# atenpas/agile_grasp

Measured on AMD Instinct MI355X. Metric: grasp hypotheses/sec on 300k-pt cloud @2000 samples, higher is better.
Workload: dtype f64

## Files before the change

### agile_grasp_amd/csrc/agh_internal.h

```cpp
#pragma once

#include <hip/hip_runtime.h>
#include <stdint.h>

#include <string>
#include <vector>

#include "agh.h"

namespace agh
{

constexpr int kBboxBlocks = 128;
constexpr int kCountBlocks = 2048;
constexpr int kGridMargin = 2;
constexpr int kCellCap = 1 << 21;
constexpr int kCellStride = kCellCap + 4;
constexpr int kMaxRows = 128;
constexpr int kNumSums = 37;
constexpr int kSumStride = 40;
constexpr int kSlots = 8;
constexpr int kImageWords = 250;
constexpr int kBigListGrid = 512;
constexpr int kSweepWg4MinSamples = 4096;
constexpr int64_t kNormalsChunk = 16384;

struct GridDesc
{
  double mn[3];
  double cell;
  double inv_cell;
  int dim[3];
  int ncell;
  unsigned open;
  unsigned ticket;
};

constexpr int kMaxClouds = 64;
struct GridView
{
  const GridDesc* desc;
  const int* cell_start;
  const float4* sorted;
  const int* cloud_off;
  int n_clouds;
};

struct HandGeom
{
  double finger_width, hand_outer_diameter, hand_depth, hand_height, init_bite;
  double cam_origin[2][3];
  double cos_a[8], sin_a[8];
  double fs[20];
  double thr[40];
  int n_thr;
  int lo_idx[20], hi_idx[20];
  double depths[16];
  double backs[16];
  double boxy[16];
  int n_depths;
  double cos_antipodal;
  double xlut_lo, xlut_scale;
  double ylut_lo, ylut_scale;
  unsigned char xlut[1024];
  unsigned char ylut[64];
  int x_probes, y_probes;
};
constexpr int kLutProbe = 4;

struct HogTablesDev
{
  float mag0[9], mag1[9];
  int bin0[9], bin1[9];
  alignas(16) float coef[9][12];
  int pix_x[256], pix_y[256];
  float pix_wcell[256][4];
};

enum SampleStatus : int
{
  kStatusOk = 0,
  kStatusOverflow = 1,
  kStatusDegenerate = 2,
  kStatusRows = 3,
  kStatusBadIndex = 4,
  kStatusSkipped = 5
};
constexpr int32_t kSampleSkip = INT32_MIN;
constexpr int kBigCap = 4096;
constexpr int kHugeCap = 6144;
constexpr int64_t kHugeEntries = 1ll << 21;

constexpr unsigned long long kVoxMaxWords = 1ull << 28;
struct VoxDesc
{
  unsigned mn_enc[2][3], mx_enc[2][3];
  double mn[2][3];
  int dim[2][3];
  unsigned long long bits[2], word_ofs[2], n_words;
  long long n_kept[2], n_vox[2];
  int error;
};
struct VoxWorkspace
{
  double lo[3], hi[3];
};

struct Comm;

struct HostMirror
{
  agh_hypothesis* rec;
  int64_t cap;
  int64_t* hdr;
};

struct LocalizeState
{
  bool active = false;
  bool repeated = false;
  bool deferred = false;
  bool classify = false, with_sequential = false, explicit_samples = false;
  int64_t S = 0, nv = 0;
  int32_t min_inliers = 0;
  double min_length = 0.0, x1 = 0.0, x2 = 0.0;
  agh_localize_params lp{};
  const float* d_raw = nullptr;
  int64_t dev_stride = 0, n_raw = 0;
  bool staged = false;
  const float* staged_src = nullptr;
  int64_t staged_stride = 0, staged_n = 0;
};

struct PlaneState;

struct Ctx
{
  agh_params p;
  HandGeom geom;
  int device = 0;
  hipStream_t stream = nullptr;
  hipEvent_t copy_done = nullptr;
  hipEvent_t copy_gate = nullptr;
  hipEvent_t xyz_copied = nullptr;
  bool cam_copy_on_copy_stream = false;
  hipStream_t copy_stream = nullptr;
  bool copy_stream_failed = false;
  std::string err;

  int64_t n = 0;
  const float* d_xyz = nullptr;
  int64_t stride_floats = 3;
  const int32_t* d_cam = nullptr;
  float* own_xyz = nullptr;
  int32_t* own_cam = nullptr;
  int64_t own_cap = 0;
  int64_t own_cap_floats = 0;
  int32_t* d_idx_own = nullptr;
  int64_t idx_cap = 0;
  uint8_t* h_pin = nullptr;
  int64_t h_pin_samples = 0, h_pin_records = 0;
  HostMirror mirror{ nullptr, 0, nullptr };
  uint8_t* h_pin_handles = nullptr;
  int64_t h_pin_handles_cap = 0;
  bool handles_sequential = false;
  uint8_t* h_pin_keep = nullptr;
  int64_t h_pin_keep_cap = 0;

  VoxDesc* d_vox_desc = nullptr;
  uint8_t* d_vox_code = nullptr;
  int* d_vox_blk = nullptr;
  int* d_vox_blk2 = nullptr;
  long long* d_vox_total = nullptr;
  unsigned* d_vox_bitmap = nullptr;
  int64_t vox_bitmap_cap = 0;
// ... 650 lines not shown
```

### agile_grasp_amd/csrc/api.hip

```cpp
#include "agh_internal.h"

#include <algorithm>
#include <atomic>
#include <cmath>
#include <cstdio>
#include <cstdlib>
#include <cstring>

using namespace agh;


namespace
{
thread_local std::string g_create_error;
std::atomic<int32_t> g_epoch{ 0 };
}

namespace agh
{
int32_t next_epoch()
{
  int32_t e;
  do
    e = (int32_t) ((uint32_t) g_epoch.fetch_add(1) + 1u) & 0x7fffffff;
// ... 960 lines not shown
  }
  int* h_counts = reinterpret_cast<int*>(c->h_pin_handles);
  agh_hypothesis* h_hands = reinterpret_cast<agh_hypothesis*>(c->h_pin_handles + 256);
  agh_handle* h_handles = reinterpret_cast<agh_handle*>(h_hands + c->h_pin_handles_cap);
  int32_t* h_idx = reinterpret_cast<int32_t*>(h_handles + c->h_pin_handles_cap);
  if (n_hands > 0)
  {
    std::memcpy(h_hands, hands, sizeof(agh_hypothesis) * (size_t) n_hands);
    HIPCHK(c, hipMemcpyAsync(c->d_h_hands, h_hands, sizeof(agh_hypothesis) * n_hands, hipMemcpyHostToDevice, c->stream));
  }
  const HandleMirror hm{ h_handles, (int) c->h_pin_handles_cap, h_idx, (int) c->h_pin_handles_cap, h_counts };
  for (int attempt = 0; attempt < 2; attempt++)
  {
    h_counts[0] = h_counts[1] = h_counts[2] = h_counts[3] = 0;
    timing_begin(c, c->stream);
    const bool with_sequential = c->handles_sequential;
    const int rc = handle_search(c, n_hands, x1, x2, min_inliers, min_length, c->stream, hm, with_sequential);
    timing_mark(c, "handle_search", c->stream);
    if (rc != AGH_OK)
    {
      c->err = "handle search launch failed";
      return rc;
    }
    HIPCHK(c, hipStreamSynchronize(c->stream));
    const bool declined = h_counts[3] != 0;
    c->handles_sequential = declined;
    if (!declined || with_sequential)
      break;
  }
  const int* counts = h_counts;
  if (counts[2])
  {
    c->err = "agh_find_handles: a seed hand has more than 2048 inliers";
    return AGH_ERR_CAPACITY;
  }
  *n_handles_out = counts[0];
  if (counts[0] > handle_cap || counts[1] > idx_cap)
  {
    c->err = "agh_find_handles: output buffers too small";
    return AGH_ERR_CAPACITY;
  }
  if (counts[0] > 0)
  {
    std::memcpy(handles_out, h_handles, sizeof(agh_handle) * (size_t) counts[0]);
    std::memcpy(inlier_idx_out, h_idx, sizeof(int32_t) * (size_t) counts[1]);
  }
  return AGH_OK;
}

int agh_get_cloud(agh_ctx* ctx, float* xyz_out, int32_t* cam_out, int64_t cap)
{
  if (!ctx || cap < 0)
    return AGH_ERR_INVALID_ARGUMENT;
  Ctx* c = &ctx->c;
  if (refuse_mid_chain(c, "agh_get_cloud"))
    return AGH_ERR_STATE;
  if (!c->has_cloud)
  {
    c->err = "agh_get_cloud: no cloud set";
    return AGH_ERR_NO_CLOUD;
  }
  HIPCHK(c, hipSetDevice(c->device));
  HIPCHK(c, hipDeviceSynchronize());
  const int64_t k = std::min<int64_t>(cap, c->n);
  if (k > 0 && xyz_out)
    HIPCHK(c, hipMemcpy2D(xyz_out, 12, c->d_xyz, (size_t) c->stride_floats * 4, 12, (size_t) k, hipMemcpyDeviceToHost));
  if (k > 0 && cam_out)
  {
    if (c->d_cam)
      HIPCHK(c, hipMemcpy(cam_out, c->d_cam, sizeof(int32_t) * k, hipMemcpyDeviceToHost));
    else
      std::memset(cam_out, 0, sizeof(int32_t) * k);
  }
  return (int) std::min<int64_t>(c->n, 0x7fffffff);
}

int agh_find_hands_device(agh_ctx* ctx, const int32_t* d_sample_idx, int64_t n_samples, int calculates_antipodal,
  agh_hypothesis* d_out, int64_t cap, int64_t* d_n_out, void* hip_stream)
{
  if (!ctx)
    return AGH_ERR_INVALID_ARGUMENT;
  Ctx* c = &ctx->c;
  if (refuse_mid_chain(c, "agh_find_hands"))
    return AGH_ERR_STATE;
  if (!c->has_cloud)
  {
    c->err = "agh_find_hands: no cloud set";
    return AGH_ERR_NO_CLOUD;
  }
  if (n_samples < 0 || n_samples > (1 << 24) || (n_samples > 0 && (!d_sample_idx || !d_out)) || !d_n_out || cap < 0)
  {
    c->err = "agh_find_hands: bad arguments";
    return AGH_ERR_INVALID_ARGUMENT;
  }
  HIPCHK(c, hipSetDevice(c->device));
  hipStream_t st = hip_stream ? (hipStream_t) hip_stream : c->stream;
  HIPCHK(c, order_after_cloud(c, st));
  const int64_t S = n_samples;
  const int64_t chunk = kNormalsChunk;
  int rc = ensure_call_buffers(c, std::max<int64_t>(S, calculates_antipodal ? std::min<int64_t>(c->n, chunk) : 0));
  if (rc != AGH_OK)
    return rc;
  const bool rand_mode = c->p.normals_mode == AGH_NORMALS_RAND50;
  if (rand_mode)
  {
    rc = ensure_draws(c, 50 * (S + (calculates_antipodal ? c->n : 0)), st);
    if (rc != AGH_OK)
      return rc;
  }
  timing_begin(c, st);
  c->zero_flags_pending = true;
  c->last_s = S;
  c->epoch = next_epoch();
  c->last_nout = -1;
  c->last_cap = cap;
  c->d_out_last = d_out;
  c->d_nout_last = d_n_out;
  if (S == 0 || c->n == 0)
  {
    HIPCHK(c, hipMemsetAsync(c->d_flags, 0, 8 * sizeof(int32_t), st));
    c->zero_flags_pending = false;
    HIPCHK(c, hipMemsetAsync(d_n_out, 0, sizeof(int64_t), st));
    c->last_s = 0;
    return AGH_OK;
  }
  if (calculates_antipodal)
  {
    if (c->n > c->normals_cap)
    {
      if ((rc = dev_alloc(c, &c->d_normals, (size_t) c->n * 3)))
        return rc;
      c->normals_cap = c->n;
    }
    HIPCHK(c, hipMemsetAsync(c->d_normals, 0, sizeof(double) * 3 * c->n, st));
    if ((rc = normals_pass(c, 0, c->n, st)) != AGH_OK)
    {
      c->err = "normals pass launch failed";
      return rc;
    }
    c->has_normals = true;
  }
  rc = taubin_frames(c, d_sample_idx, S, c->p.nn_radius_taubin, c->d_frames, c->d_nt, calculates_antipodal != 0, st);
  if (rc != AGH_OK)
  {
    c->err = "taubin launch failed";
    return rc;
  }
  if (c->debug_stop_moments || (c->debug_stop_frame && c->debug_stop_frame < 5))
  {
    HIPCHK(c, hipMemsetAsync(d_n_out, 0, sizeof(int64_t), st));
    return AGH_OK;
  }
#ifdef AGH_DEBUG_HOOKS
  if (std::getenv("AGH_DEBUG_CLOCKS") && !c->d_dbg && hipMalloc((void**) &c->d_dbg, sizeof(long long) * 8 * c->s_cap) != hipSuccess)
    c->d_dbg = nullptr;
#endif
  rc = hand_sweep(c, d_sample_idx, S, calculates_antipodal != 0, st);
  if (rc != AGH_OK)
  {
    c->err = "hand sweep launch failed";
    return rc;
  }
  if (c->debug_stop_sweep && c->debug_stop_sweep < 10)
  {
    HIPCHK(c, hipMemsetAsync(d_n_out, 0, sizeof(int64_t), st));
    return AGH_OK;
  }
  rc = compact_hypotheses(c, S, d_out, cap, d_n_out, st);
  if (rc != AGH_OK)
  {
    c->err = "compaction launch failed";
    return rc;
  }
  return AGH_OK;
}


static int check_flags(Ctx* c, hipStream_t st)
{
  int32_t flags[8];
  HIPCHK(c, hipMemcpyAsync(flags, c->d_flags, sizeof(flags), hipMemcpyDeviceToHost, st));
  HIPCHK(c, hipStreamSynchronize(st));
  return flags_to_status(c, flags);
}

extern "C++" int flags_to_status(Ctx* c, const int32_t* flags_in)
{
  int32_t flags[1] = { flags_in[0] };
  if (flags[0] & kFlagSharded)
  {
    flags[0] &= ~1;
    if (flags[0] & kFlagShardPeerNoCloud)
    {
      c->err = "a rank of the communicator holds no cloud (agh_set_cloud* on every rank first); no list";
      return AGH_ERR_NO_CLOUD;
    }
    if (flags[0] & kFlagShardPeerFailed)
    {
      c->err = "a rank of the communicator could not do its share of the call (its own agh_last_error says why); no list";
      return AGH_ERR_STATE;
    }
    if (flags[0] & kFlagShardHard)
    {
      c->err = "the Taubin neighbourhoods (r = nn_radius_taubin) of more than 4096 points of one launch hold more than 2^21 points in "
               "all; voxelise the cloud (localization.cpp:43) or reduce the radii";
      return AGH_ERR_CAPACITY;
    }
    if (flags[0] & (kFlagShardRetry | kFlagShardRetryHuge))
    {
      c->big_classes = true;
      if (flags[0] & kFlagShardRetryHuge)
        c->huge_classes = true;
      c->err = "a Taubin neighbourhood exceeds the capacity classes launched so far; the contexts of the communicator now launch "
               "the larger classes as well: repeat the call";
      return AGH_ERR_RETRY;
    }
  }
  if ((flags[0] & 1) && !c->big_classes)
  {
    c->big_classes = true;
    c->err = "a Taubin neighbourhood exceeds the first capacity class; the context now launches the larger classes as "
             "well: repeat the call";
    return AGH_ERR_RETRY;
  }
  if ((flags[0] & 1) && !c->huge_classes)
  {
    c->huge_classes = true;
    c->err = "a Taubin neighbourhood exceeds 4096 points; the context now launches the 6144 class as well: repeat the call";
    return AGH_ERR_RETRY;
  }
  if (flags[0] & 1)
  {
    c->err = "the Taubin neighbourhoods (r = nn_radius_taubin) of more than 4096 points of one launch hold more than 2^21 points in "
             "all (the pool of the classes beyond the LDS-resident ones); voxelise the cloud (localization.cpp:43) or reduce the radii";
    return AGH_ERR_CAPACITY;
  }
  if ((flags[0] & 2) && !(flags[0] & 16))
  {
    c->err = "output buffer too small for the hypotheses found";
    return AGH_ERR_CAPACITY;
  }
  if (flags[0] & 4)
  {
    c->err = "a sample index is outside the cloud";
    return AGH_ERR_INVALID_ARGUMENT;
  }
  if (flags[0] & 16)
  {
    c->shard_full_exchange = true;
    c->err = "a rank found more hypotheses than its exchange segment holds; the context now exchanges full-size segments: "
             "repeat the call";
    return AGH_ERR_RETRY;
  }
  return AGH_OK;
}

int agh_find_hands(agh_ctx* ctx, const int32_t* sample_idx, int64_t n_samples, int calculates_antipodal,
  agh_hypothesis* out, int64_t cap, int64_t* n_out)
{
  if (!ctx || !n_out)
    return AGH_ERR_INVALID_ARGUMENT;
  Ctx* c = &ctx->c;
  if (refuse_mid_chain(c, "agh_find_hands"))
    return AGH_ERR_STATE;
  *n_out = 0;
  if (!c->has_cloud)
  {
    c->err = "agh_find_hands: no cloud set";
    return AGH_ERR_NO_CLOUD;
  }
  if (n_samples < 0 || (n_samples > 0 && !sample_idx) || cap < 0 || (cap > 0 && !out))
  {
    c->err = "agh_find_hands: bad arguments";
    return AGH_ERR_INVALID_ARGUMENT;
  }
  for (int64_t i = 0; i < n_samples; i++)
    if (sample_idx[i] < 0 || sample_idx[i] >= c->n)
    {
      c->err = "agh_find_hands: sample index out of range";
      return AGH_ERR_INVALID_ARGUMENT;
    }
  HIPCHK(c, hipSetDevice(c->device));
  int rc = ensure_call_buffers(c, std::max<int64_t>(n_samples, calculates_antipodal ? std::min<int64_t>(c->n, kNormalsChunk) : 0));
  if (rc != AGH_OK)
    return rc;
  if (n_samples > c->idx_cap || !c->d_idx_own)
  {
    if ((rc = dev_alloc(c, &c->d_idx_own, (size_t) std::max<int64_t>(n_samples, 1024))))
      return rc;
    c->idx_cap = std::max<int64_t>(n_samples, 1024);
  }
  int32_t* d_idx = c->d_idx_own;
  if ((rc = ensure_host_staging(c, n_samples, std::min<int64_t>(c->s_cap * 8, kMirrorMaxRecords))) != AGH_OK)
    return rc;
  int64_t* hdr = reinterpret_cast<int64_t*>(c->h_pin);
  int32_t* h_idx = reinterpret_cast<int32_t*>(c->h_pin + kPinHeaderBytes);
  agh_hypothesis* h_rec = reinterpret_cast<agh_hypothesis*>(c->h_pin + kPinHeaderBytes + pin_round(c->h_pin_samples * 4));
  if (n_samples > 0)
  {
    std::memcpy(h_idx, sample_idx, sizeof(int32_t) * (size_t) n_samples);
    HIPCHK(c, hipMemcpyAsync(d_idx, h_idx, sizeof(int32_t) * n_samples, hipMemcpyHostToDevice, c->stream));
  }
  int64_t n = 0;
  for (int attempt = 0; attempt < 3; attempt++)
  {
    if ((rc = ensure_call_buffers(c, std::max<int64_t>(n_samples, calculates_antipodal ? std::min<int64_t>(c->n, kNormalsChunk) : 0))) != AGH_OK)
      return rc;
    hdr[0] = -1;
    hdr[1] = 0;
    c->mirror = HostMirror{ h_rec, c->h_pin_records, hdr };
    rc = agh_find_hands_device(ctx, d_idx, n_samples, calculates_antipodal, c->d_out_own, c->s_cap * 8, c->d_nout,
      c->stream);
    c->mirror = HostMirror{ nullptr, 0, nullptr };
    if (rc == AGH_OK)
    {
      HIPCHK(c, hipStreamSynchronize(c->stream));
      int32_t flags[8] = { 0, 0, 0, 0, 0, 0, 0, 0 };
      if (hdr[0] >= 0)
      {
        n = hdr[0];
        flags[0] = (int32_t) hdr[1] | (n > c->s_cap * 8 ? 2 : 0);
      }
      else
      {
        HIPCHK(c, hipMemcpy(flags, c->d_flags, sizeof(flags), hipMemcpyDeviceToHost));
        HIPCHK(c, hipMemcpy(&n, c->d_nout, sizeof(int64_t), hipMemcpyDeviceToHost));
      }
      rc = flags_to_status(c, flags);
    }
    else
      (void) hipStreamSynchronize(c->stream);
    if (rc != AGH_ERR_RETRY)
      break;
  }
  if (rc != AGH_OK)
    return rc;
  c->last_nout = n;
  *n_out = n;
  if (n > cap)
  {
    c->err = "output buffer too small for the hypotheses found";
    return AGH_ERR_CAPACITY;
  }
  const int64_t from_pin = hdr[0] >= 0 ? std::min<int64_t>(n, c->h_pin_records) : 0;
  if (from_pin > 0)
    std::memcpy(out, h_rec, sizeof(agh_hypothesis) * (size_t) from_pin);
  if (n > from_pin)
    HIPCHK(c, hipMemcpy(out + from_pin, c->d_out_own + from_pin, sizeof(agh_hypothesis) * (size_t) (n - from_pin), hipMemcpyDeviceToHost));
  return AGH_OK;
}

int agh_synchronize(agh_ctx* ctx)
{
  if (!ctx)
    return AGH_ERR_INVALID_ARGUMENT;
  Ctx* c = &ctx->c;
  HIPCHK(c, hipSetDevice(c->device));
  HIPCHK(c, hipDeviceSynchronize());
  if (c->loc.active)
    return AGH_OK;
#ifdef AGH_DEBUG_HOOKS
  if (c->d_dbg && c->last_s > 0 && std::getenv("AGH_DEBUG_CLOCKS"))
  {
    std::vector<long long> h((size_t) c->last_s * 8);
    if (hipMemcpy(h.data(), c->d_dbg, h.size() * 8, hipMemcpyDeviceToHost) == hipSuccess)
      if (FILE* f = std::fopen(std::getenv("AGH_DEBUG_CLOCKS"), "wb"))
      {
        std::fwrite(h.data(), 8, h.size(), f);
        std::fclose(f);
      }
  }
#endif
  const int rc = check_flags(c, c->stream);
  if (rc == AGH_OK && c->last_nout < 0 && c->d_nout_last)
  {
    int64_t n = 0;
    if (hipMemcpy(&n, c->d_nout_last, sizeof(int64_t), hipMemcpyDeviceToHost) == hipSuccess)
      c->last_nout = std::min<int64_t>(n, c->last_cap);
    else
      (void) hipGetLastError();
  }
  return rc;
}

int agh_get_epoch(agh_ctx* ctx, int32_t* epoch, int64_t* n_hyp)
{
  if (!ctx)
    return AGH_ERR_INVALID_ARGUMENT;
  if (refuse_mid_chain(&ctx->c, "agh_get_epoch"))
    return AGH_ERR_STATE;
  if (epoch)
    *epoch = ctx->c.epoch;
  if (n_hyp)
    *n_hyp = ctx->c.last_nout;
  return AGH_OK;
}

int agh_get_frames(agh_ctx* ctx, agh_frame* out, int64_t cap)
{
  if (!ctx || !out)
    return AGH_ERR_INVALID_ARGUMENT;
  Ctx* c = &ctx->c;
  if (refuse_mid_chain(c, "agh_get_frames"))
    return AGH_ERR_STATE;
  const int64_t n = std::min<int64_t>(cap, c->last_s);
  HIPCHK(c, hipDeviceSynchronize());
  if (n > 0)
    HIPCHK(c, hipMemcpy(out, c->d_frames, sizeof(agh_frame) * n, hipMemcpyDeviceToHost));
  return (int) n;
}

int agh_get_neighbor_counts(agh_ctx* ctx, int32_t* n_taubin, int32_t* n_hands, int64_t cap)
{
  if (!ctx)
    return AGH_ERR_INVALID_ARGUMENT;
  Ctx* c = &ctx->c;
  if (refuse_mid_chain(c, "agh_get_neighbor_counts"))
    return AGH_ERR_STATE;
  const int64_t n = std::min<int64_t>(cap, c->last_s);
  HIPCHK(c, hipDeviceSynchronize());
  if (n > 0 && n_taubin)
    HIPCHK(c, hipMemcpy(n_taubin, c->d_nt, sizeof(int32_t) * n, hipMemcpyDeviceToHost));
  if (n > 0 && n_hands)
  {
    if (ball_counts(c, n, c->stream) != AGH_OK)
    {
      c->err = "k_ball_count launch failed";
      return AGH_ERR_HIP;
    }
    HIPCHK(c, hipStreamSynchronize(c->stream));
  }
  if (n > 0 && n_hands)
    HIPCHK(c, hipMemcpy(n_hands, c->d_nh, sizeof(int32_t) * n, hipMemcpyDeviceToHost));
  return (int) n;
}

int agh_get_normals(agh_ctx* ctx, double* normals, int64_t cap_points)
{
  if (!ctx || !normals)
    return AGH_ERR_INVALID_ARGUMENT;
  Ctx* c = &ctx->c;
  if (refuse_mid_chain(c, "agh_get_normals"))
    return AGH_ERR_STATE;
  if (!c->has_normals)
  {
    c->err = "no normals: the last agh_find_hands call did not use calculates_antipodal";
    return AGH_ERR_STATE;
  }
  const int64_t n = std::min<int64_t>(cap_points, c->n);
  HIPCHK(c, hipDeviceSynchronize());
  if (n > 0)
    HIPCHK(c, hipMemcpy(normals, c->d_normals, sizeof(double) * 3 * n, hipMemcpyDeviceToHost));
  return (int) n;
}

int agh_set_profile(agh_ctx* ctx, int32_t level)
{
  if (!ctx || level < 0 || level > 3)
    return AGH_ERR_INVALID_ARGUMENT;
  Ctx* c = &ctx->c;
  if (refuse_mid_chain(c, "agh_set_profile"))
    return AGH_ERR_STATE;
  HIPCHK(c, hipSetDevice(c->device));
  HIPCHK(c, hipDeviceSynchronize());
  c->p.profile = level;
  c->prof_calls = 0;
  c->ev_used = 0;
  c->ev_name.clear();
  return AGH_OK;
}

int agh_get_timing(agh_ctx* ctx, agh_timing* out)
{
  if (!ctx || !out)
    return AGH_ERR_INVALID_ARGUMENT;
  Ctx* c = &ctx->c;
  std::memset(out, 0, sizeof(*out));
  std::memset(c->timing_counts, 0, sizeof(c->timing_counts));
  if (!c->p.profile || c->ev_used < 2)
    return AGH_OK;
  HIPCHK(c, hipEventSynchronize(c->ev[c->ev_used - 1]));
  int k = 0;
  for (int i = 1; i < c->ev_used; i++)
  {
    if (std::strcmp(c->ev_name[i], "start") == 0)
      continue;
    float ms = 0.f;
    if (hipEventElapsedTime(&ms, c->ev[i - 1], c->ev[i]) != hipSuccess)
      ms = 0.f;
    int slot = -1;
    for (int j = 0; j < k; j++)
      if (std::strcmp(out->name[j], c->ev_name[i]) == 0)
        slot = j;
    if (slot < 0)
    {
      if (k >= AGH_TIMING_SLOTS)
        continue;
      slot = k++;
      out->name[slot] = c->ev_name[i];
    }
    out->ms[slot] += ms;
    c->timing_counts[slot]++;
    out->total_ms += ms;
  }
  out->n = k;
  c->ev_used = 0;
  c->ev_name.clear();
  return AGH_OK;
}

int agh_get_timing_counts(agh_ctx* ctx, int32_t* counts, int32_t cap)
{
  if (!ctx || !counts || cap < 0)
    return AGH_ERR_INVALID_ARGUMENT;
  for (int i = 0; i < cap && i < AGH_TIMING_SLOTS; i++)
    counts[i] = ctx->c.timing_counts[i];
  return AGH_OK;
// ... 32 lines not shown
```

### agile_grasp_amd/csrc/taubin.hip

```cpp
#include "agh_internal.h"

#include <cstring>
#include <utility>

#include "taubin_eigen.h"

namespace agh
{

constexpr int kSortBins = 256;
constexpr int kChunk = 56;

template <int CAP>
__device__ __forceinline__ void taubin_moments_sample(const int s, GridView gv, const float* __restrict__ xyz, int64_t stride,
  const int32_t* __restrict__ samples, int S, float r2f, double rpad, int first_class, double* __restrict__ sums,
  int32_t* __restrict__ nt, int32_t* __restrict__ status, float4* __restrict__ nbr, int64_t nbr_stride, int debug_stop,
  int n_points, int32_t* __restrict__ zero_flags, int32_t* __restrict__ scloud, long long* __restrict__ dbg,
  int32_t* __restrict__ ovf_out)
{
#ifdef AGH_DEBUG_HOOKS
#define AGH_MSTAMP(i) do { if (dbg && threadIdx.x == 0) dbg[(int64_t) blockIdx.x * 8 + (i)] = wall_clock64(); } while (0)
  long long mt_prod = 0, mt_cons = 0, mt_wait = 0, mt_last = 0;
#define AGH_MLAP(acc) do { if (dbg) { const long long now_ = wall_clock64(); acc += now_ - mt_last; mt_last = now_; } } while (0)
#else
// ... 605 lines not shown
    for (int u = 0; u < kPer; u++)
      pos[u] = bin[u] >= 0 ? atomicAdd(&hist[bin[u]], 1) : 0;
#pragma unroll
    for (int u = 0; u < kPer; u++)
      if (bin[u] >= 0)
        order[pos[u]] = base + u * kT + tid;
  }
}

constexpr int kSweepBlock = 32, kSweepBlocksMax = 1024;
__device__ void sweep_order_block(const int* __restrict__ weight, int S, int* __restrict__ order2, int* bw )
{
  const int B = (S + kSweepBlock - 1) / kSweepBlock;
  if (B > kSweepBlocksMax)
    return;
  const int tid = threadIdx.x;
  __syncthreads();
  for (int b = tid; b < B; b += 256)
  {
    int w = 0;
    const int i0 = b * kSweepBlock, i1 = min(S, i0 + kSweepBlock);
    for (int i = i0; i < i1; i++)
      w += weight[i];
    bw[b] = w;
  }
  __syncthreads();
  const int last_size = S - (B - 1) * kSweepBlock;
  int rank_last = 0;
  for (int q = 0; q < B - 1; q++)
    rank_last += bw[q] >= bw[B - 1] ? 1 : 0;
  for (int b = tid; b < B; b += 256)
  {
    const int wb = bw[b];
    int rank = 0;
    for (int q = 0; q < B; q++)
      rank += (bw[q] > wb || (bw[q] == wb && q < b)) ? 1 : 0;
    const int pos = rank * kSweepBlock - (rank > rank_last ? kSweepBlock - last_size : 0);
    const int size = b == B - 1 ? last_size : kSweepBlock;
    for (int k = 0; k < size; k++)
      order2[pos + k] = b * kSweepBlock + k;
  }
}

__device__ void draw_offsets_wave(const int32_t* __restrict__ nt, int S, int32_t* __restrict__ draw_ofs,
  int32_t* __restrict__ total_io)
{
  constexpr int kPer = 16;
  const int lane = threadIdx.x;
  int carry = *total_io;
  for (int c0 = 0; c0 < S; c0 += 64 * kPer)
  {
    const int i0 = c0 + lane * kPer;
    int v[kPer], sum = 0;
#pragma unroll
    for (int u = 0; u < kPer; u++)
    {
      v[u] = (i0 + u < S && nt[i0 + u] > 50) ? 50 : 0;
      sum += v[u];
    }
    const int inc = wave_incl_scan_i32(sum);
    int run = carry + inc - sum;
#pragma unroll
    for (int u = 0; u < kPer; u++)
    {
      if (i0 + u < S)
        draw_ofs[i0 + u] = run;
      run += v[u];
    }
    carry += __builtin_amdgcn_readlane(inc, 63);
  }
  if (lane == 0)
    *total_io = carry;
}

template <int LPS>
__global__ __launch_bounds__(256) void k_taubin_eigen(const double* __restrict__ sums, const int32_t* __restrict__ nt,
  const int32_t* __restrict__ status, int S, double* __restrict__ eig, int32_t* __restrict__ flags,
  const int* __restrict__ weight, int* __restrict__ order, int32_t* __restrict__ draw_ofs, int32_t* __restrict__ draw_total_io,
  int* __restrict__ order_sweep)
{
  __shared__ int hist[kOrderBins];
  __shared__ int wave_tot[4];
  static_assert(kSweepBlocksMax <= kOrderBins, "the sweep's block weights reuse the histogram");
  const int n_solver_groups = (S * LPS + 255) / 256;
  if (order && (int) blockIdx.x == n_solver_groups)
  {
    sample_order_block(weight, S, order, hist, wave_tot);
    return;
  }
  if (order && (int) blockIdx.x == n_solver_groups + 1)
  {
    if (order_sweep)
      sweep_order_block(weight, S, order_sweep, hist);
    return;
  }
  if ((int) blockIdx.x >= n_solver_groups + (order ? 2 : 0))
  {
    if (threadIdx.x < 64)
      draw_offsets_wave(nt, S, draw_ofs, draw_total_io);
    return;
  }
  const int s = (int) (blockIdx.x * 256 + threadIdx.x) / LPS;
  const bool writer = (threadIdx.x % LPS) == 0;
  if (s >= S)
    return;
  double sv[kNumSums];
#pragma unroll
  for (int k = 0; k < kNumSums; k++)
    sv[k] = sums[(int64_t) s * kSumStride + k];
  const int st_ = status[s];
  if (writer && (st_ == kStatusOverflow || st_ == kStatusRows))
    atomicOr(&flags[0], 1);
  if (writer && st_ == kStatusBadIndex)
    atomicOr(&flags[0], 4);
  const bool live = st_ == kStatusOk && nt[s] > 0;
#pragma unroll
  for (int k = 0; k < kNumSums; k++)
    sv[k] = live ? sv[k] : 0.0;
  double v[10];
  const double lambda = taubin_smallest_eigenpair<LPS>(sv, live ? (double) nt[s] : 1.0, v);
  if (!writer)
    return;
  double* out = eig + (int64_t) s * 12;
#pragma unroll
  for (int k = 0; k < 10; k++)
    out[k] = live ? ((k >= 3 && k < 6) ? v[k] * 0.5 : v[k]) : 0.0;
  out[10] = live ? lambda : 0.0;
  out[11] = live ? 1.0 : 0.0;
}

__device__ const double kMultinomial6[28] = { 1.0, 6.0, 6.0, 15.0, 30.0, 15.0, 20.0, 60.0, 60.0, 20.0, 15.0, 60.0, 90.0, 60.0, 15.0, 6.0, 30.0, 60.0, 60.0, 30.0, 6.0, 1.0, 6.0, 15.0, 20.0, 15.0, 6.0, 1.0 };

__device__ __forceinline__ double wave_max_f64_(double v)
{
  v = fmax(v, xor_partner_f64<32>(v));
  v = fmax(v, xor_partner_f64<16>(v));
  v = fmax(v, xor_partner_f64<8>(v));
  v = fmax(v, xor_partner_f64<4>(v));
  v = fmax(v, xor_partner_f64<2>(v));
  v = fmax(v, xor_partner_f64<1>(v));
  return v;
}

template <int CAP, int THREADS>
__global__ __launch_bounds__(THREADS, (CAP == 1152 && THREADS == 256) ? 5 : ((CAP == 64 && THREADS == 256) ? 8 : 1)) void k_taubin_frame(const float4* __restrict__ nbr, int64_t nbr_stride,
  const int32_t* __restrict__ nt, const double* __restrict__ eig, const int32_t* __restrict__ status,
  const float* __restrict__ xyz, int64_t stride, const int32_t* __restrict__ samples, int S, int rand_mode,
  const int32_t* __restrict__ draw_ofs, const int32_t* __restrict__ draws, double cam0x, double cam0y, double cam0z,
  double cam1x, double cam1y, double cam1z, agh_frame* __restrict__ frames, double* __restrict__ normals_out, int nmin, int debug_stop,
  const int* __restrict__ order, long long* __restrict__ dbg, const float4* __restrict__ pool_sorted,
  const long long* __restrict__ huge_base, const int32_t* __restrict__ ovf_list)
{
#ifdef AGH_DEBUG_HOOKS
#define AGH_FSTAMP(i, t) do { if (dbg && threadIdx.x == (t)) dbg[(int64_t) (order ? order[blockIdx.x] : (int) blockIdx.x) * 8 + (i)] = wall_clock64(); } while (0)
#else
#define AGH_FSTAMP(i, t) do { } while (0)
#endif
  AGH_FSTAMP(0, 0);
  __shared__ double nx[CAP], ny[CAP], nz[CAP];
  __shared__ int camcnt[2];
  __shared__ int next_col;
  __shared__ double sM3[6];
  __shared__ double sAxis[3];
  constexpr int NW = THREADS / 64;
  __shared__ double wbest[NW];
  __shared__ int wbest_j[NW];
  __shared__ double sT[NW][28];
  __shared__ double sW[28];
  __shared__ double wmax_s[NW];
  __shared__ unsigned short cand[CAP];
  __shared__ int ncand;
  __shared__ int bar3cnt;
#ifdef AGH_FRAME_PAD
  __shared__ int pad_[AGH_FRAME_PAD / 4];
  if (threadIdx.x == 0 && nmin == -12345)
    pad_[blockIdx.x % (AGH_FRAME_PAD / 4)] = 1;
#endif

  const int tid = threadIdx.x, lane = tid & 63, wave = tid >> 6;
  auto body = [&](const int s) {
  const int n = nt[s];
  const double* ev = eig + (int64_t) s * 12;
  const bool ok = status[s] == kStatusOk && ev[11] != 0.0;
  const int ks_class = (rand_mode && n > 50) ? 50 : n;
  if (ok ? (ks_class <= nmin || ks_class > CAP) : (nmin != 0))
    return;
  const bool valid = ok;
  const bool bad_index = status[s] == kStatusBadIndex || status[s] == kStatusSkipped;
  const float* qp = xyz + (int64_t) (bad_index ? 0 : samples[s]) * stride;
  if (!valid)
  {
    if (tid == 0)
    {
      agh_frame f;
      for (int k = 0; k < 3; k++)
      {
        f.sample[k] = bad_index ? 0.0 : (double) qp[k];
        f.normal[k] = f.axis[k] = f.binormal[k] = 0.0;
      }
      for (int k = 0; k < 10; k++)
        f.params[k] = 0.0;
      f.eigenvalue = 0.0;
      f.n_nb = n;
      f.majority_cam = 0;
      f.max_index = 0;
      f.valid = 0;
      frames[s] = f;
    }
    return;
  }
  const double a = ev[0], b = ev[1], c = ev[2];
  const double d = 2.0 * ev[3], e = 2.0 * ev[4], f = 2.0 * ev[5];
  const double g = ev[6], h = ev[7], i9 = ev[8];
  AGH_FSTAMP(1, 0);
  const bool sub = rand_mode && n > 50;
  const int ks = sub ? 50 : n;
  if (tid < 2)
    camcnt[tid] = 0;
  if (tid == 0)
  {
    next_col = 0;
    ncand = 0;
    bar3cnt = 0;
  }
  __syncthreads();
  const float4* nb = (huge_base && huge_base[s] >= 0) ? pool_sorted + huge_base[s] : nbr + (int64_t) s * nbr_stride;
  int cam1 = 0;
  for (int t = tid; t < ks; t += THREADS)
  {
    const int pick = sub ? (draws[draw_ofs[s] + t] % n) : t;
    const float4 p = nb[pick];
    const double x = (double) p.x, y = (double) p.y, z = (double) p.z;
    const double fx = (((2.0 * a) * x + d * y) + f * z) + g;
    const double fy = (((2.0 * b) * y + d * x) + e * z) + h;
    const double fz = (((2.0 * c) * z + e * y) + f * x) + i9;
    const double mag = sqrt((fx * fx + fy * fy) + fz * fz);
    nx[t] = fx / mag;
    ny[t] = fy / mag;
    nz[t] = fz / mag;
    cam1 += (int) (__float_as_uint(p.w) & 1u);
  }
  cam1 = wave_allsum_i32(cam1);
  if (lane == 0 && cam1)
    atomicAdd(&camcnt[1], cam1);
  __syncthreads();
  AGH_FSTAMP(2, 0);
  if (debug_stop == 1)
    return;
  constexpr bool kSplit = NW == 4;
  const bool use3 = kSplit && ks > 64;
  constexpr int ET = kSplit ? THREADS - 64 : THREADS;
  constexpr int ENW = kSplit ? NW - 1 : NW;
  const int et = kSplit ? tid - 64 : tid, ew = kSplit ? wave - 1 : wave;
  int bar_phase = 0;
  auto wait3 = [&](int target) {
    while (__hip_atomic_load(&bar3cnt, __ATOMIC_RELAXED, __HIP_MEMORY_SCOPE_WORKGROUP) < target)
      __builtin_amdgcn_s_sleep(1);
    __threadfence_block();
  };
  auto ebar = [&]() {
    if (kSplit)
    {
      bar_phase++;
      __threadfence_block();
      __builtin_amdgcn_wave_barrier();
      if (lane == 0)
        __hip_atomic_fetch_add(&bar3cnt, 1, __ATOMIC_RELAXED, __HIP_MEMORY_SCOPE_WORKGROUP);
      wait3(3 * bar_phase);
    }
    else
      __syncthreads();
  };
  auto m3_and_axis = [&]() {
    double m[6] = { 0.0, 0.0, 0.0, 0.0, 0.0, 0.0 };
    if (!(debug_stop == 5 || debug_stop == 7))
      for (int t = lane; t < ks; t += 64)
      {
        const double x = nx[t], y = ny[t], z = nz[t];
        m[0] += x * x;
        m[1] += x * y;
        m[2] += x * z;
        m[3] += y * y;
        m[4] += y * z;
        m[5] += z * z;
      }
#pragma unroll
    for (int k = 0; k < 6; k++)
    {
      m[k] = wave_allsum_f64(m[k]);
      if (lane == 0)
        sM3[k] = m[k];
    }
    __builtin_amdgcn_wave_barrier();
    __threadfence_block();
    if (lane == 0)
    {
      const double m3[6] = { sM3[0], sM3[1], sM3[2], sM3[3], sM3[4], sM3[5] };
      double ax[3] = { 1.0, 0.0, 0.0 };
      if (!(debug_stop == 6 || debug_stop == 7))
        smallest_eigvec3(m3, ax);
      sAxis[0] = ax[0];
      sAxis[1] = ax[1];
      sAxis[2] = ax[2];
    }
  };
  constexpr bool kSmallCols = CAP <= 128;
  const bool small_cols = kSmallCols && ks <= 64;
  double small_best = -1.0;
  int small_best_j = 0x7fffffff;
  if (!kSmallCols && ks <= 64)
  {
    for (int j = tid; j < ks; j += THREADS)
      cand[j] = (unsigned short) j;
    if (tid == 0)
      ncand = ks;
  }
  else if (small_cols)
  {
    if (tid == 0)
      ncand = 0;
    if (wave == NW - 1)
    {
      const int j = lane < ks ? lane : 0;
      const double jx = nx[j], jy = ny[j], jz = nz[j];
      double s0 = 0.0, s1 = 0.0, s2 = 0.0;
#pragma unroll 1
      for (int b = 0; b < 8; b++)
      {
        const int br = ((b & 1) << 2) | (b & 2) | ((b & 4) >> 2);
        double stk[4];
#pragma unroll
        for (int k = 0; k < 8; k++)
        {
          const int i = ((((k & 1) << 2) | (k & 2) | ((k & 4) >> 2)) << 3) | br;
          const int ii = i < ks ? i : 0;
          const double gdot = (nx[ii] * jx + ny[ii] * jy) + nz[ii] * jz;
          const double g2 = gdot * gdot;
          double v = i < ks ? (g2 * g2) * g2 : 0.0;
          int depth = __builtin_popcount(k);
#pragma unroll
          for (int m = 0; m < 3; m++)
            if (((k >> m) & 1) && ((k & ((1 << m) - 1)) == ((1 << m) - 1)))
            {
              depth--;
              v = stk[depth] + v;
            }
          stk[depth] = v;
        }
        double v = stk[0];
        if (b & 1)
        {
          v = s0 + v;
          if (b & 2)
          {
            v = s1 + v;
            if (b & 4)
              v = s2 + v;
            else
              s2 = v;
          }
          else
            s1 = v;
        }
        else
          s0 = v;
        if (b == 7)
          s0 = v;
      }
      if (lane < ks)
      {
        small_best = s0;
        small_best_j = lane;
      }
    }
  }
  else if (CAP <= 64)
    ;
  else if (kSplit && wave == 0)
    m3_and_axis();
  else
  {
    const double mult_et = kMultinomial6[et < 28 ? et : 0];
    {
      double T[28];
  #pragma unroll
      for (int k = 0; k < 28; k++)
        T[k] = 0.0;
      for (int t = et; t < ks; t += ET)
      {
        const double x = nx[t], y = ny[t], z = nz[t];
        double px[7], py[7], pz[7];
        px[0] = py[0] = pz[0] = 1.0;
  #pragma unroll
        for (int k = 1; k < 7; k++)
        {
          px[k] = px[k - 1] * x;
          py[k] = py[k - 1] * y;
          pz[k] = pz[k - 1] * z;
        }
        int k = 0;
  #pragma unroll
        for (int a = 6; a >= 0; a--)
  #pragma unroll
          for (int b = 6 - a; b >= 0; b--)
          {
            T[k] = fma(px[a], py[b] * pz[6 - a - b], T[k]);
            k++;
          }
      }
      double R[32];
  #pragma unroll
      for (int k = 0; k < 32; k++)
        R[k] = k < 28 ? T[k] : 0.0;
  #pragma unroll
      for (int half = 16, o = 32; half >= 1; half >>= 1, o >>= 1)
      {
        const bool upper = (lane & o) != 0;
  #pragma unroll
        for (int k = 0; k < half; k++)
        {
          const double send = upper ? R[k] : R[k + half];
          const double keep = upper ? R[k + half] : R[k];
          R[k] = keep + __shfl_xor(send, o);
        }
      }
      R[0] = R[0] + __shfl_xor(R[0], 1);
      if ((lane & 1) == 0 && (lane >> 1) < 28)
        sT[ew][lane >> 1] = R[0];
    }
    AGH_FSTAMP(3, 64);
    ebar();
    if (et < 28)
    {
      double tsum = sT[0][et];
      for (int w = 1; w < ENW; w++)
        tsum = tsum + sT[w][et];
      sW[et] = tsum * mult_et;
    }
    ebar();
    constexpr int EST = (CAP + ET - 1) / ET;
    double est[EST];
    double est_max = -1.0;
    {
      double W[28];
  #pragma unroll
      for (int k = 0; k < 28; k++)
        W[k] = sW[k];
  #pragma unroll
      for (int m = 0; m < EST; m++)
      {
        const int j = et + ET * m;
        double e_ = -2.0;
        if (j < ks)
// ... 615 lines not shown
```

### agile_grasp_amd/csrc/taubin_eigen.h

```cpp
#pragma once
#include <hip/hip_runtime.h>

#include "agh_internal.h"

#ifndef AGH_EIG_STAMP0
#define AGH_EIG_TEMPLATE template <int LPS>
#define AGH_EIG_STAMP0
#define AGH_EIG_STAMP1
#define AGH_EIG_STAMP2
#define AGH_EIG_STAMP3
#define AGH_EIG_STAMP4
#define AGH_EIG_STAMP5
#define AGH_EIG_STAMP6
#endif

namespace agh
{

constexpr double kDeflateTol = 0x1p-40;
constexpr double kPivMin = 0x1p-500;
constexpr int kBisectSteps = 56;

__device__ __forceinline__ double pivot_floor(double x) { return (fabs(x) >= kPivMin) ? x : kPivMin; }

// ... 197 lines not shown
  for (int i = 0; i < 9; i++)
    d[i] = C[i][i];
#pragma unroll
  for (int i = 0; i < 8; i++)
    e2[i] = e[i] * e[i];
  AGH_EIG_STAMP3;
  double lo = 0.0, hi = 0.0;
  bool first = true;
#pragma unroll
  for (int i = 0; i < 9; i++)
  {
    const double r = ((i > 0) ? fabs(e[i > 0 ? i - 1 : 0]) : 0.0) + ((i < 8) ? fabs(e[i < 8 ? i : 7]) : 0.0);
    const double g0 = d[i] - r;
    const bool take = !defl[i];
    lo = (take && (first || g0 < lo)) ? g0 : lo;
    hi = (take && (first || d[i] < hi)) ? d[i] : hi;
    first = first && !take;
  }
  auto below_at = [&](double x) -> bool {
    double pm2 = 1.0, pm1 = d[0] - x;
    int sgn = __double2hiint(pm1);
#pragma unroll
    for (int i = 1; i < 9; i++)
    {
      const double pi = fma(d[i] - x, pm1, -(e2[i - 1] * pm2));
      sgn |= __double2hiint(pi);
      pm2 = pm1;
      pm1 = pi;
    }
    return sgn < 0;
  };
  if (LPS == 1)
  {
#pragma unroll 1
    for (int it = 0; it < kBisectSteps; it++)
    {
      const double mid = fma(hi - lo, 0.5, lo);
      const bool below = below_at(mid);
      hi = below ? mid : hi;
      lo = below ? lo : mid;
    }
  }
  else
  {
    static_assert(LPS == 1 || LPS == 8, "one lane per sample, or eight");
    const int q = (int) (threadIdx.x & 7);
    const int gshift = (int) (threadIdx.x & 63 & ~7);
    int left = kBisectSteps;
#pragma unroll 1
    while (left > 0)
    {
      const int levels = left >= 3 ? 3 : left;
      double nlo = lo, nhi = hi;
      const int depth = q >= 4 ? 2 : (q >= 2 ? 1 : 0);
#pragma unroll
      for (int l = 0; l < 2; l++)
        if (l < depth)
        {
          const double m = fma(nhi - nlo, 0.5, nlo);
          const bool right = ((q >> (depth - 1 - l)) & 1) != 0;
          nlo = right ? m : nlo;
          nhi = right ? nhi : m;
        }
      const double mid = fma(nhi - nlo, 0.5, nlo);
      const bool below = below_at(mid);
      const unsigned verdicts = (unsigned) (__ballot(below) >> gshift) & 0xffu;
      int node = 1;
#pragma unroll
      for (int l = 0; l < 3; l++)
        if (l < levels)
        {
          const double m = fma(hi - lo, 0.5, lo);
          const bool b = ((verdicts >> node) & 1u) != 0;
          hi = b ? m : hi;
          lo = b ? lo : m;
          node = 2 * node + (b ? 0 : 1);
        }
      left -= levels;
    }
  }
  const double sigma = lo;
  double Dp[9], Dm[9], lf[8], ub[8];
  Dp[0] = pivot_floor(d[0] - sigma);
#pragma unroll
  for (int i = 0; i < 8; i++)
  {
    lf[i] = e[i] / Dp[i];
    Dp[i + 1] = pivot_floor(fma(-lf[i], e[i], d[i + 1] - sigma));
  }
  Dm[8] = pivot_floor(d[8] - sigma);
#pragma unroll
  for (int i = 7; i >= 0; i--)
  {
    ub[i] = e[i] / Dm[i + 1];
    Dm[i] = pivot_floor(fma(-ub[i], e[i], d[i] - sigma));
  }
  int ks = -1;
  double gmin = 0.0;
#pragma unroll
  for (int k = 0; k < 9; k++)
  {
    const double gk = fabs((Dp[k] + Dm[k]) - (d[k] - sigma));
    const bool take = !defl[k] && (ks < 0 || gk < gmin);
    ks = take ? k : ks;
    gmin = take ? gk : gmin;
  }
  double z[9];
  {
    double zl[10];
    zl[9] = 0.0;
#pragma unroll
    for (int i = 8; i >= 0; i--)
      zl[i] = (i == ks) ? 1.0 : ((i < ks) ? -(lf[i < 8 ? i : 7] * zl[i + 1]) : 0.0);
    double zu = 0.0;
#pragma unroll
    for (int i = 0; i < 9; i++)
    {
      zu = (i == ks) ? 1.0 : ((i > ks) ? -(ub[i > 0 ? i - 1 : 0] * zu) : 0.0);
      z[i] = (i <= ks) ? zl[i] : zu;
    }
  }
  AGH_EIG_STAMP5;
#pragma unroll
  for (int k = 6; k >= 0; k--)
  {
    double s2 = 0.0;
#pragma unroll
    for (int i = k + 1; i < 9; i++)
      s2 = fma(C[i][k], z[i], s2);
    s2 = s2 * RH[k];
#pragma unroll
    for (int i = k + 1; i < 9; i++)
      z[i] = fma(-s2, C[i][k], z[i]);
  }
#pragma unroll
  for (int i = 8; i >= 0; i--)
  {
    double s2 = z[i];
#pragma unroll
    for (int k = i + 1; k < 9; k++)
      s2 = fma(-L[k][i], v[k], s2);
    v[i] = s2 * rinv[i];
  }
  AGH_EIG_STAMP6;
  double bv = 0.0;
#pragma unroll
  for (int k = 0; k < 9; k++)
    bv = fma(b[k], v[k], bv);
  v[9] = -(bv / n);
  return sigma;
}


__device__ __forceinline__ void smallest_eigvec3(const double (&m)[6], double (&axis)[3])
{
  const double x0 = m[1], x1 = m[2];
  const double sg = fma(x1, x1, x0 * x0);
  const double rt = sqrt(sg);
  const double g = (x0 >= 0.0) ? -rt : rt;
  const double h = fma(-x0, g, sg);
  const bool live = h > 0.0;
  const double rh = live ? 1.0 / h : 0.0;
  const double u1 = live ? x0 - g : 0.0, u2 = live ? x1 : 0.0;
  const double p1 = fma(m[4], u2, m[3] * u1) * rh;
  const double p2 = fma(m[5], u2, m[4] * u1) * rh;
  const double kk = (fma(u2, p2, u1 * p1) * rh) * 0.5;
  const double q1 = fma(-kk, u1, p1), q2 = fma(-kk, u2, p2);
  const double d0 = m[0], d1 = fma(-q1, u1, fma(-u1, q1, m[3])), d2 = fma(-q2, u2, fma(-u2, q2, m[5]));
  const double e0 = live ? g : x0, e1 = fma(-q2, u1, fma(-u2, q1, m[4]));
  const double e20 = e0 * e0, e21 = e1 * e1;
  const double r0 = fabs(e0), r1 = fabs(e0) + fabs(e1), r2 = fabs(e1);
  double lo = d0 - r0, hi = d0;
  lo = (d1 - r1 < lo) ? d1 - r1 : lo;
  lo = (d2 - r2 < lo) ? d2 - r2 : lo;
  hi = (d1 < hi) ? d1 : hi;
  hi = (d2 < hi) ? d2 : hi;
#pragma unroll 1
  for (int it = 0; it < kBisectSteps; it++)
  {
    const double mid = fma(hi - lo, 0.5, lo);
    const double s1 = d0 - mid;
    const double s2 = fma(d1 - mid, s1, -e20);
    const double s3 = fma(d2 - mid, s2, -(e21 * s1));
    const bool below = ((__double2hiint(s1) | __double2hiint(s2)) | __double2hiint(s3)) < 0;
    hi = below ? mid : hi;
    lo = below ? lo : mid;
  }
  const double sigma = lo;
  const double Dp0 = pivot_floor(d0 - sigma);
  const double lf0 = e0 / Dp0;
  const double Dp1 = pivot_floor(fma(-lf0, e0, d1 - sigma));
  const double lf1 = e1 / Dp1;
  const double Dp2 = pivot_floor(fma(-lf1, e1, d2 - sigma));
  const double Dm2 = pivot_floor(d2 - sigma);
  const double ub1 = e1 / Dm2;
  const double Dm1 = pivot_floor(fma(-ub1, e1, d1 - sigma));
  const double ub0 = e0 / Dm1;
  const double Dm0 = pivot_floor(fma(-ub0, e0, d0 - sigma));
  const double g0 = fabs((Dp0 + Dm0) - (d0 - sigma)), g1 = fabs((Dp1 + Dm1) - (d1 - sigma)), g2 = fabs((Dp2 + Dm2) - (d2 - sigma));
  int ks = 0;
  double gmin = g0;
  ks = (g1 < gmin) ? 1 : ks;
  gmin = (g1 < gmin) ? g1 : gmin;
  ks = (g2 < gmin) ? 2 : ks;
  double z0, z1, z2;
  if (ks == 0)
  {
    z0 = 1.0;
    z1 = -(ub0 * z0);
    z2 = -(ub1 * z1);
  }
  else if (ks == 1)
  {
    z1 = 1.0;
    z0 = -(lf0 * z1);
    z2 = -(ub1 * z1);
  }
  else
  {
    z2 = 1.0;
    z1 = -(lf1 * z2);
    z0 = -(lf0 * z1);
  }
  const double sdot = fma(u2, z2, u1 * z1) * rh;
  const double y0 = z0, y1 = fma(-sdot, u1, z1), y2 = fma(-sdot, u2, z2);
  const double nn = sqrt(fma(y2, y2, fma(y1, y1, y0 * y0)));
  axis[0] = y0 / nn;
  axis[1] = y1 / nn;
  axis[2] = y2 / nn;
}

}
```

Baseline: 4.210 million.

## Parallelize 3x3 eigenvalue bisection across a wave using ballot tree search

The 3x3 smallest-eigenvector bisection no longer runs on lane 0 alone. All 64 lanes now evaluate a 6-level bisection tree in parallel, and ballot plus readlane pick the winning interval, so the serial 56-step loop shrinks to about 10 wave iterations. The shared-memory staging of the moment sums, with its wave barrier and fence, is dropped because every lane already holds the reduced sums. Debug clock slots are widened to 16 per frame. The risk is extra per-lane ALU and readlane traffic; this is a small piece of the frame kernel.

```diff
diff --git a/agile_grasp_amd/csrc/agh_internal.h b/agile_grasp_amd/csrc/agh_internal.h
--- a/agile_grasp_amd/csrc/agh_internal.h
+++ b/agile_grasp_amd/csrc/agh_internal.h
@@ -21,6 +21,7 @@
 constexpr int kSumStride = 40;
 constexpr int kSlots = 8;
 constexpr int kImageWords = 250;
+constexpr int kFrameClockSlots = 16;
 constexpr int kBigListGrid = 512;
 constexpr int kSweepWg4MinSamples = 4096;
 constexpr int64_t kNormalsChunk = 16384;
diff --git a/agile_grasp_amd/csrc/api.hip b/agile_grasp_amd/csrc/api.hip
--- a/agile_grasp_amd/csrc/api.hip
+++ b/agile_grasp_amd/csrc/api.hip
@@ -1136,7 +1136,7 @@
     return AGH_OK;
   }
 #ifdef AGH_DEBUG_HOOKS
-  if (std::getenv("AGH_DEBUG_CLOCKS") && !c->d_dbg && hipMalloc((void**) &c->d_dbg, sizeof(long long) * 8 * c->s_cap) != hipSuccess)
+  if (std::getenv("AGH_DEBUG_CLOCKS") && !c->d_dbg && hipMalloc((void**) &c->d_dbg, sizeof(long long) * kFrameClockSlots * c->s_cap) != hipSuccess)
     c->d_dbg = nullptr;
 #endif
   rc = hand_sweep(c, d_sample_idx, S, calculates_antipodal != 0, st);
@@ -1346,7 +1346,8 @@
 #ifdef AGH_DEBUG_HOOKS
   if (c->d_dbg && c->last_s > 0 && std::getenv("AGH_DEBUG_CLOCKS"))
   {
-    std::vector<long long> h((size_t) c->last_s * 8);
+    const char* k = std::getenv("AGH_DEBUG_CLOCKS_KERNEL");
+    std::vector<long long> h((size_t) c->last_s * ((k && !std::strcmp(k, "frame")) ? kFrameClockSlots : 8));
     if (hipMemcpy(h.data(), c->d_dbg, h.size() * 8, hipMemcpyDeviceToHost) == hipSuccess)
       if (FILE* f = std::fopen(std::getenv("AGH_DEBUG_CLOCKS"), "wb"))
       {
diff --git a/agile_grasp_amd/csrc/taubin.hip b/agile_grasp_amd/csrc/taubin.hip
--- a/agile_grasp_amd/csrc/taubin.hip
+++ b/agile_grasp_amd/csrc/taubin.hip
@@ -781,7 +781,7 @@
   const long long* __restrict__ huge_base, const int32_t* __restrict__ ovf_list)
 {
 #ifdef AGH_DEBUG_HOOKS
-#define AGH_FSTAMP(i, t) do { if (dbg && threadIdx.x == (t)) dbg[(int64_t) (order ? order[blockIdx.x] : (int) blockIdx.x) * 8 + (i)] = wall_clock64(); } while (0)
+#define AGH_FSTAMP(i, t) do { if (dbg && threadIdx.x == (t)) dbg[(int64_t) (order ? order[blockIdx.x] : (int) blockIdx.x) * kFrameClockSlots + (i)] = wall_clock64(); } while (0)
 #else
 #define AGH_FSTAMP(i, t) do { } while (0)
 #endif
@@ -789,7 +789,6 @@
   __shared__ double nx[CAP], ny[CAP], nz[CAP];
   __shared__ int camcnt[2];
   __shared__ int next_col;
-  __shared__ double sM3[6];
   __shared__ double sAxis[3];
   constexpr int NW = THREADS / 64;
   __shared__ double wbest[NW];
@@ -915,19 +914,13 @@
       }
 #pragma unroll
     for (int k = 0; k < 6; k++)
-    {
       m[k] = wave_allsum_f64(m[k]);
-      if (lane == 0)
-        sM3[k] = m[k];
-    }
-    __builtin_amdgcn_wave_barrier();
-    __threadfence_block();
+    AGH_FSTAMP(8, 0);
+    double ax[3] = { 1.0, 0.0, 0.0 };
+    if (!(debug_stop == 6 || debug_stop == 7))
+      smallest_eigvec3_wave(m, ax);
     if (lane == 0)
     {
-      const double m3[6] = { sM3[0], sM3[1], sM3[2], sM3[3], sM3[4], sM3[5] };
-      double ax[3] = { 1.0, 0.0, 0.0 };
-      if (!(debug_stop == 6 || debug_stop == 7))
-        smallest_eigvec3(m3, ax);
       sAxis[0] = ax[0];
       sAxis[1] = ax[1];
       sAxis[2] = ax[2];
diff --git a/agile_grasp_amd/csrc/taubin_eigen.h b/agile_grasp_amd/csrc/taubin_eigen.h
--- a/agile_grasp_amd/csrc/taubin_eigen.h
+++ b/agile_grasp_amd/csrc/taubin_eigen.h
@@ -373,41 +373,57 @@
 }
 
 
-__device__ __forceinline__ void smallest_eigvec3(const double (&m)[6], double (&axis)[3])
-{
+struct Eig3Tri
+{
+  double d0, d1, d2, e0, e1, e20, e21, u1, u2, rh, lo, hi;
+};
+
+__device__ __forceinline__ Eig3Tri eig3_tridiagonal(const double (&m)[6])
+{
+  Eig3Tri t;
   const double x0 = m[1], x1 = m[2];
   const double sg = fma(x1, x1, x0 * x0);
   const double rt = sqrt(sg);
   const double g = (x0 >= 0.0) ? -rt : rt;
   const double h = fma(-x0, g, sg);
   const bool live = h > 0.0;
-  const double rh = live ? 1.0 / h : 0.0;
-  const double u1 = live ? x0 - g : 0.0, u2 = live ? x1 : 0.0;
-  const double p1 = fma(m[4], u2, m[3] * u1) * rh;
-  const double p2 = fma(m[5], u2, m[4] * u1) * rh;
-  const double kk = (fma(u2, p2, u1 * p1) * rh) * 0.5;
+  t.rh = live ? 1.0 / h : 0.0;
+  t.u1 = live ? x0 - g : 0.0;
+  t.u2 = live ? x1 : 0.0;
+  const double u1 = t.u1, u2 = t.u2;
+  const double p1 = fma(m[4], u2, m[3] * u1) * t.rh;
+  const double p2 = fma(m[5], u2, m[4] * u1) * t.rh;
+  const double kk = (fma(u2, p2, u1 * p1) * t.rh) * 0.5;
   const double q1 = fma(-kk, u1, p1), q2 = fma(-kk, u2, p2);
-  const double d0 = m[0], d1 = fma(-q1, u1, fma(-u1, q1, m[3])), d2 = fma(-q2, u2, fma(-u2, q2, m[5]));
-  const double e0 = live ? g : x0, e1 = fma(-q2, u1, fma(-u2, q1, m[4]));
-  const double e20 = e0 * e0, e21 = e1 * e1;
-  const double r0 = fabs(e0), r1 = fabs(e0) + fabs(e1), r2 = fabs(e1);
-  double lo = d0 - r0, hi = d0;
-  lo = (d1 - r1 < lo) ? d1 - r1 : lo;
-  lo = (d2 - r2 < lo) ? d2 - r2 : lo;
-  hi = (d1 < hi) ? d1 : hi;
-  hi = (d2 < hi) ? d2 : hi;
-#pragma unroll 1
-  for (int it = 0; it < kBisectSteps; it++)
-  {
-    const double mid = fma(hi - lo, 0.5, lo);
-    const double s1 = d0 - mid;
-    const double s2 = fma(d1 - mid, s1, -e20);
-    const double s3 = fma(d2 - mid, s2, -(e21 * s1));
-    const bool below = ((__double2hiint(s1) | __double2hiint(s2)) | __double2hiint(s3)) < 0;
-    hi = below ? mid : hi;
-    lo = below ? lo : mid;
-  }
-  const double sigma = lo;
+  t.d0 = m[0];
+  t.d1 = fma(-q1, u1, fma(-u1, q1, m[3]));
+  t.d2 = fma(-q2, u2, fma(-u2, q2, m[5]));
+  t.e0 = live ? g : x0;
+  t.e1 = fma(-q2, u1, fma(-u2, q1, m[4]));
+  t.e20 = t.e0 * t.e0;
+  t.e21 = t.e1 * t.e1;
+  const double r0 = fabs(t.e0), r1 = fabs(t.e0) + fabs(t.e1), r2 = fabs(t.e1);
+  double lo = t.d0 - r0, hi = t.d0;
+  lo = (t.d1 - r1 < lo) ? t.d1 - r1 : lo;
+  lo = (t.d2 - r2 < lo) ? t.d2 - r2 : lo;
+  hi = (t.d1 < hi) ? t.d1 : hi;
+  hi = (t.d2 < hi) ? t.d2 : hi;
+  t.lo = lo;
+  t.hi = hi;
+  return t;
+}
+
+__device__ __forceinline__ bool eig3_below(const Eig3Tri& t, double x)
+{
+  const double s1 = t.d0 - x;
+  const double s2 = fma(t.d1 - x, s1, -t.e20);
+  const double s3 = fma(t.d2 - x, s2, -(t.e21 * s1));
+  return ((__double2hiint(s1) | __double2hiint(s2)) | __double2hiint(s3)) < 0;
+}
+
+__device__ __forceinline__ void eig3_vector(const Eig3Tri& t, double sigma, double (&axis)[3])
+{
+  const double d0 = t.d0, d1 = t.d1, d2 = t.d2, e0 = t.e0, e1 = t.e1;
   const double Dp0 = pivot_floor(d0 - sigma);
   const double lf0 = e0 / Dp0;
   const double Dp1 = pivot_floor(fma(-lf0, e0, d1 - sigma));
@@ -443,12 +459,61 @@
     z1 = -(lf1 * z2);
     z0 = -(lf0 * z1);
   }
-  const double sdot = fma(u2, z2, u1 * z1) * rh;
-  const double y0 = z0, y1 = fma(-sdot, u1, z1), y2 = fma(-sdot, u2, z2);
+  const double sdot = fma(t.u2, z2, t.u1 * z1) * t.rh;
+  const double y0 = z0, y1 = fma(-sdot, t.u1, z1), y2 = fma(-sdot, t.u2, z2);
   const double nn = sqrt(fma(y2, y2, fma(y1, y1, y0 * y0)));
   axis[0] = y0 / nn;
   axis[1] = y1 / nn;
   axis[2] = y2 / nn;
 }
 
-}
+__device__ __forceinline__ void smallest_eigvec3(const double (&m)[6], double (&axis)[3])
+{
+  const Eig3Tri t = eig3_tridiagonal(m);
+  double lo = t.lo, hi = t.hi;
+#pragma unroll 1
+  for (int it = 0; it < kBisectSteps; it++)
+  {
+    const double mid = fma(hi - lo, 0.5, lo);
+    const bool below = eig3_below(t, mid);
+    hi = below ? mid : hi;
+    lo = below ? lo : mid;
+  }
+  eig3_vector(t, lo, axis);
+}
+
+__device__ __forceinline__ void smallest_eigvec3_wave(const double (&m)[6], double (&axis)[3])
+{
+  const Eig3Tri t = eig3_tridiagonal(m);
+  double lo = t.lo, hi = t.hi;
+  const int q = (int) (threadIdx.x & 63);
+  const int depth = q ? 31 - __builtin_clz((unsigned) q) : 0;
+  constexpr int kLevels = 6;
+#pragma unroll 1
+  for (int left = kBisectSteps; left > 0; left -= kLevels)
+  {
+    const int levels = left >= kLevels ? kLevels : left;
+    double nlo = lo, nhi = hi;
+#pragma unroll
+    for (int l = 0; l < kLevels - 1; l++)
+      if (l < depth)
+      {
+        const double mm = fma(nhi - nlo, 0.5, nlo);
+        const bool right = ((q >> (depth - 1 - l)) & 1) != 0;
+        nlo = right ? mm : nlo;
+        nhi = right ? nhi : mm;
+      }
+    const double mid = fma(nhi - nlo, 0.5, nlo);
+    const bool below = eig3_below(t, mid);
+    const unsigned long long verdicts = __ballot(below);
+    int node = 1;
+    for (int l = 0; l < levels - 1; l++)
+      node = 2 * node + (((verdicts >> node) & 1ull) ? 0 : 1);
+    const double clo = below ? nlo : mid, chi = below ? mid : nhi;
+    lo = __hiloint2double(__builtin_amdgcn_readlane(__double2hiint(clo), node), __builtin_amdgcn_readlane(__double2loint(clo), node));
+    hi = __hiloint2double(__builtin_amdgcn_readlane(__double2hiint(chi), node), __builtin_amdgcn_readlane(__double2loint(chi), node));
+  }
+  eig3_vector(t, lo, axis);
+}
+
+}
```

Result: no change. 4.225 million (median of 6 runs) (+0.4%).
